# Lalwaniamisha789/Implementation-of-Neural-LDPC-Decoders-with-Degree-Specific-Weight-Sharing-and-RCQ-Quantization

Measured on AMD Instinct MI355X. Metric: decoded codewords/sec at fixed iters; achieved HBM GB/s vs peak, higher is better.
Workload: dtype f32; 1 GPU; (1998,1512) IRA code, BasicMinSumDecoder factor=0.7, fp32, 10 iterations, batch 65536/GPU, SNR 2.0 dB, fixed-iteration flooding decode; graph=ira_1998_1512, n=1998, m=486, edges=6587, batch_per_gpu=65536, global_batch=65536, parallelism=dp1, collective=none

## Files before the change

implementation-of-neural-ldpc-decoders-with-degree-specific-weight-sharing-and-rcq-quantization_amd/_native.py:

```python

from __future__ import annotations

import ctypes as C
import os
import subprocess
import threading
from typing import Optional

import numpy as np

_HERE = os.path.dirname(os.path.abspath(__file__))
LIB_NAME = "libldpc_hip.so"
LIB_PATH = os.environ.get("LDPC_HIP_LIB") or os.path.join(_HERE, LIB_NAME)
CSRC = os.path.join(_HERE, "csrc")
HEADER = os.path.join(os.path.dirname(_HERE), "include", "ldpc_hip.h")
DEBUG_HEADER = os.path.join(os.path.dirname(_HERE), "include", "ldpc_hip_debug.h")

LDPC_F32, LDPC_F64 = 0, 1
C2V_NMS, C2V_RCQ, C2V_OMS = 0, 1, 2
MODE_AUTO, MODE_STREAM, MODE_RESIDENT, MODE_SWEEPS, MODE_GATHER, MODE_PAIR = 0, 1, 2, 3, 4, 5
SCHED_FLOODING, SCHED_LAYERED_REF, SCHED_LAYERED = 0, 1, 2

HIPCC_FLAGS = ["--offload-arch=gfx950", "-O3", "-std=c++17", "-fPIC", "-shared",
               "-ffp-contract=off",
# ... 49 lines not shown
    tmp = target + ".tmp%d" % os.getpid()
    cmd = [hipcc] + HIPCC_FLAGS + [f"-D{d}" for d in defines] + [f"-DLDPC_SRC_HASH={want}", "-o", tmp, srcs[0]]
    res = subprocess.run(cmd, capture_output=True, text=True)
    if verbose or res.returncode != 0:
        print(" ".join(cmd))
        print(res.stdout + res.stderr)
    if res.returncode != 0:
        try:
            os.unlink(tmp)
        except OSError:
            pass
        raise NativeEngineError("hipcc failed:\n" + res.stderr[-4000:])
    os.replace(tmp, target)
    return target


class DecoderDesc(C.Structure):
    _fields_ = [("dtype", C.c_int32), ("c2v_form", C.c_int32), ("iters", C.c_int32),
                ("n_beta_slots", C.c_int32), ("beta", C.c_void_p), ("beta_slot", C.c_void_p),
                ("n_alpha_slots", C.c_int32), ("alpha", C.c_void_p), ("alpha_slot", C.c_void_p),
                ("n_levels", C.c_int32), ("n_quantizers", C.c_int32), ("thresholds", C.c_void_p),
                ("q_of_iter", C.c_void_p),
                ("n_oms_alpha_slots", C.c_int32), ("oms_alpha", C.c_void_p), ("oms_alpha_slot", C.c_void_p),
                ("schedule", C.c_int32)]


PRODUCT_EXPORTS = ("ldpc_graph_create", "ldpc_graph_destroy", "ldpc_graph_info", "ldpc_decoder_create",
                   "ldpc_decoder_set_mode", "ldpc_decoder_info",
                   "ldpc_decoder_set_weights", "ldpc_decoder_destroy", "ldpc_decoder_workspace_bytes",
                   "ldpc_decode", "ldpc_decode_capped", "ldpc_last_error", "ldpc_abi_version", "ldpc_source_hash",
                   "ldpc_train_saved_bytes", "ldpc_train_workspace_bytes", "ldpc_decode_saving", "ldpc_backward",
                   "ldpc_train_joint_workspace_bytes", "ldpc_train_joint")
DEBUG_EXPORTS = ("ldpc_debug_sweep", "ldpc_debug_workspace_layout", "ldpc_debug_resident_c2v", "ldpc_debug_key4",
                 "ldpc_debug_compact_layout")
EXPORTS = PRODUCT_EXPORTS + DEBUG_EXPORTS

_lib = None
_lock = threading.Lock()


def load():
    global _lib
    if _lib is not None:
        return _lib
    with _lock:
        if _lib is not None:
            return _lib
        if not os.path.exists(LIB_PATH):
            raise NativeEngineError(
                f"{LIB_NAME} is not built: run `python -c 'import __graft_entry__ as g; g.build()'` "
                f"(hipcc --offload-arch=gfx950) -- there is no CPU fallback for the decode path")
        if "LDPC_HIP_LIB" not in os.environ and is_stale(LIB_PATH):
            raise NativeEngineError(
                f"{LIB_PATH} was not built from the sources in csrc/ (content hash {built_hash(LIB_PATH)} != "
                f"{source_hash()}): run `python -c 'import __graft_entry__ as g; g.build()'` -- a stale engine is never loaded")
        try:
            lib = C.CDLL(LIB_PATH)
        except OSError as e:
            raise NativeEngineError(f"cannot load {LIB_PATH}: {e}") from e
        vp, i32, i64 = C.c_void_p, C.c_int32, C.c_int64
        lib.ldpc_graph_create.restype = C.c_int
        lib.ldpc_graph_create.argtypes = [C.POINTER(vp), i32, i32, i32, vp, vp]
        lib.ldpc_graph_destroy.restype = None
        lib.ldpc_graph_destroy.argtypes = [vp]
        lib.ldpc_graph_info.restype = C.c_int
        lib.ldpc_graph_info.argtypes = [vp, vp]
        lib.ldpc_decoder_create.restype = C.c_int
        lib.ldpc_decoder_create.argtypes = [C.POINTER(vp), vp, C.POINTER(DecoderDesc)]
        lib.ldpc_decoder_set_mode.restype = C.c_int
        lib.ldpc_decoder_set_mode.argtypes = [vp, i32]
        lib.ldpc_decoder_info.restype = C.c_int
        lib.ldpc_decoder_info.argtypes = [vp, vp]
        lib.ldpc_decoder_set_weights.restype = C.c_int
        lib.ldpc_decoder_set_weights.argtypes = [vp, vp, vp, vp, vp]
        lib.ldpc_decoder_destroy.restype = None
        lib.ldpc_decoder_destroy.argtypes = [vp]
        lib.ldpc_decoder_workspace_bytes.restype = C.c_size_t
        lib.ldpc_decoder_workspace_bytes.argtypes = [vp, i64]
        lib.ldpc_decode.restype = C.c_int
        lib.ldpc_decode.argtypes = [vp, vp, i64, i32, vp, vp, vp, vp, vp, vp, C.c_size_t, vp]
        lib.ldpc_decode_capped.restype = C.c_int
        lib.ldpc_decode_capped.argtypes = [vp, vp, i64, i32, i32, vp, vp, vp, vp, vp, vp, C.c_size_t, vp]
        lib.ldpc_debug_sweep.restype = C.c_int
        lib.ldpc_debug_sweep.argtypes = [vp, i64, i32, i32, vp, C.c_size_t, vp]
        lib.ldpc_debug_workspace_layout.restype = C.c_int
        lib.ldpc_debug_workspace_layout.argtypes = [vp, i64, i32, vp]
        lib.ldpc_debug_key4.restype = C.c_int
        lib.ldpc_debug_key4.argtypes = [vp, i64, C.c_float, vp, vp, vp, vp]
        lib.ldpc_debug_resident_c2v.restype = C.c_int
        lib.ldpc_debug_resident_c2v.argtypes = [vp, vp, i64, i32, i32, vp, vp, vp, vp]
        lib.ldpc_debug_compact_layout.restype = C.c_int
        lib.ldpc_debug_compact_layout.argtypes = [vp, i32, i32, i32, vp, vp, vp, vp, vp]
        lib.ldpc_train_saved_bytes.restype = C.c_size_t
        lib.ldpc_train_saved_bytes.argtypes = [vp, i64]
        lib.ldpc_train_workspace_bytes.restype = C.c_size_t
        lib.ldpc_train_workspace_bytes.argtypes = [vp, i64]
        lib.ldpc_decode_saving.restype = C.c_int
        lib.ldpc_decode_saving.argtypes = [vp, vp, i64, i32, vp, vp, vp, vp, vp, C.c_size_t, vp, C.c_size_t, vp]
        lib.ldpc_backward.restype = C.c_int
        lib.ldpc_backward.argtypes = [vp, vp, C.c_size_t, vp, i64, vp, vp, vp, vp, vp, vp, vp, C.c_size_t, vp]
        lib.ldpc_train_joint_workspace_bytes.restype = C.c_size_t
        lib.ldpc_train_joint_workspace_bytes.argtypes = [vp, i64]
        lib.ldpc_train_joint.restype = C.c_int
        lib.ldpc_train_joint.argtypes = [vp, vp, vp, i64, vp, vp, vp, vp, vp, vp, vp, vp, vp, C.c_size_t, vp]
        lib.ldpc_last_error.restype = C.c_char_p
        lib.ldpc_last_error.argtypes = []
        lib.ldpc_abi_version.restype = C.c_int
        lib.ldpc_abi_version.argtypes = []
        lib.ldpc_source_hash.restype = C.c_char_p
        lib.ldpc_source_hash.argtypes = []
        if lib.ldpc_abi_version() != 1:
            raise NativeEngineError("libldpc_hip.so ABI version mismatch")
        _lib = lib
    return _lib


def check(rc: int, what: str):
    if rc != 0:
        msg = load().ldpc_last_error().decode(errors="replace")
        if rc == -3:
            raise NotImplementedError(f"{what}: {msg}")
        if rc == -1:
            raise ValueError(f"{what}: {msg}")
        raise NativeEngineError(f"{what} failed (rc={rc}): {msg}")

# ... 4 lines not shown
```

implementation-of-neural-ldpc-decoders-with-degree-specific-weight-sharing-and-rcq-quantization_amd/csrc/ldpc_hip.hip:

```cpp
#include "ldpc_kernels.hip"
#include "ldpc_resident.hip"
#include "ldpc_train.hip"
#include "ldpc_layered.hip"

#include <algorithm>
#include <climits>
#include <mutex>
#include <set>
#include <cmath>
#include <cstdarg>
#include <cstdio>
#include <cstdlib>
#include <cstring>
#include <exception>
#include <new>
#include <vector>

#include "../../include/ldpc_hip.h"
#include "../../include/ldpc_hip_debug.h"

using namespace ldpc;

namespace {

// ... 991 lines not shown

void cpt_lane_order(std::vector<int> &var_at, const std::vector<std::vector<int>> &vs, int G)
{
    const int n = (int)vs.size() - 1;
    std::vector<int> order(var_at.size());
    for (size_t q = 0; q < var_at.size(); ++q) order[q] = var_at[q] >= 0 ? var_at[q] : n;
    LaneCost lc{vs, order, 32, 32, G == 2 ? 16 : 32, G == 2 ? 16 : 32};
    std::vector<std::vector<int>> classes(kCptMaxDv + 1);
    for (int q = 0; q < (int)order.size(); ++q) {
        const int d = (int)vs[order[q]].size();
        if (order[q] != n && d > 0 && d <= kCptMaxDv) classes[d].push_back(q);
    }
    classes.erase(std::remove_if(classes.begin(), classes.end(), [](const std::vector<int> &c) { return c.size() < 2; }),
                  classes.end());
    if (classes.empty()) return;
    uint64_t rng = 0x9E3779B97F4A7C15ull;
    auto next = [&]() { rng ^= rng << 13; rng ^= rng >> 7; rng ^= rng << 17; return rng; };
    const long trials = std::min<long>(400000, 150L * n);
    for (long it = 0; it < trials; ++it) {
        const auto &c = classes[next() % classes.size()];
        const int x = c[next() % c.size()], y = c[next() % c.size()];
        if (x / lc.wg == y / lc.wg) continue;
        const int before = lc.around(x, y);
        std::swap(order[x], order[y]);
        if (lc.around(x, y) > before) std::swap(order[x], order[y]);
    }
    for (size_t q = 0; q < var_at.size(); ++q) var_at[q] = order[q] == n ? -1 : order[q];
}

struct ResVCheck { int check, e0, dc, gs; };
int resident_layout(ldpc_decoder *d, const ldpc_decoder_desc *desc, const std::vector<ResVCheck> &vc, int mstride,
                    long long S, int G, ResidentPlan &pl, const CptLayout *cl = nullptr);
void cpt_layout(const ldpc_graph *g, const std::vector<ResVCheck> &vc, long long S, CptLayout &L);
bool cpt_geometry(const ldpc_graph *g, const std::vector<ResVCheck> &vc, long long &Sc);

bool resident_checks(const ldpc_graph *g, std::vector<ResVCheck> &vc)
{
    auto dc_real = [&](int i) { return g->h_check_ptr[i + 1] - g->h_check_ptr[i]; };
    std::vector<int> wide_ids, plain_ids;
    for (int i = 0; i < g->m; ++i) (dc_real(i) > kResSubDegreeCap ? wide_ids : plain_ids).push_back(i);
    auto group_of = [&](int i) { int k = 1; while (k * kResSubDegree < dc_real(i)) k <<= 1; return k; };
    for (int i : wide_ids)
        if (group_of(i) > 64) return false;
    std::stable_sort(wide_ids.begin(), wide_ids.end(), [&](int a, int b) { return group_of(a) > group_of(b); });
    for (int i : wide_ids) {
        const int k = group_of(i), dc = dc_real(i), base = dc / k, rem = dc % k;
        int e = g->h_check_ptr[i];
        for (int j = 0; j < k; ++j) {
            const int len = base + (j < rem ? 1 : 0);
            vc.push_back({i, e, len, k});
            e += len;
        }
    }
    std::stable_sort(plain_ids.begin(), plain_ids.end(), [&](int a, int b) { return dc_real(a) > dc_real(b); });
    for (int i : plain_ids) vc.push_back({i, g->h_check_ptr[i], dc_real(i), 1});
    return true;
}

int build_resident_plan(ldpc_decoder *d, const ldpc_decoder_desc *desc)
{
    const ldpc_graph *g = d->g;
    d->res_ok = false;
    if (g->E == 0 || g->max_dv > 8) return LDPC_OK;
    const bool f64 = d->dtype == LDPC_F64;
    if (f64 && (d->form != LDPC_C2V_NMS || !d->beta_per_check)) return LDPC_OK;
    const int n = g->n;
// ... 25 lines not shown
    }
    const long long S = (long long)max_sub * mstride;
    const int NT = blocks >= 2 ? 512 : 1024;
    if (int rc = resident_layout(d, desc, vc, mstride, S, G, d->res)) return rc;
    d->res_G = G; d->res_NT = NT;
    d->res_lds = res_lds_total((int)S, n, G, resident_alpha_floats(d), d->res.par_words);
    d->res_ok = true;

    d->resc_ok = false;
    long long Sc = 0;
    if (!f64 && G == 2 && NT == kResCptThreads && cpt_geometry(g, vc, Sc)) {
        cpt_layout(g, vc, Sc, d->resc_layout);
        if (int rc = resident_layout(d, desc, vc, kResCptStride, Sc, 2, d->resc, &d->resc_layout)) return rc;
        d->resc_lds = res_cpt_lds_total((int)Sc, 2);
        d->resc_ok = true;
    }
    return LDPC_OK;
}

bool cpt_geometry(const ldpc_graph *g, const std::vector<ResVCheck> &vc, long long &Sc)
{
    const int n = g->n, m = (int)vc.size();
    int max_sub = 0;
    for (const ResVCheck &v : vc) max_sub = std::max(max_sub, v.dc);
    if (m != g->m || m > kResCptStride || n > kResRegVars * kResCptThreads || g->max_dv > kCptMaxDv || max_sub < 1)
        return false;
    int n_top = 0;
    while (n_top < m && vc[n_top].dc == max_sub) ++n_top;
    Sc = (long long)(max_sub - 1) * kResCptStride + n_top;
    int n_hi = 0;
    for (int j = 0; j < n; ++j) n_hi += (g->h_var_ptr[j + 1] - g->h_var_ptr[j]) > 4 ? 1 : 0;
    return Sc * 2 * 4 <= 65535 && (long long)n <= Sc && n_hi <= kResCptThreads &&
           kResCptBlocks * res_cpt_lds_total((int)Sc, 2) <= kLdsBytes;
}

void cpt_layout(const ldpc_graph *g, const std::vector<ResVCheck> &vc, long long S, CptLayout &L)
{
    const int n = g->n, m = (int)vc.size();
    std::vector<int> dv(n);
    for (int j = 0; j < n; ++j) dv[j] = g->h_var_ptr[j + 1] - g->h_var_ptr[j];
    std::vector<int> slot_of_edge(g->E);
    for (int p = 0; p < m; ++p)
        for (int t = 0; t < vc[p].dc; ++t) slot_of_edge[vc[p].e0 + t] = t * kResCptStride + p;
    std::vector<std::vector<int>> vs(n + 1);
    for (int j = 0; j < n; ++j)
        for (int k = 0; k < dv[j]; ++k) vs[j].push_back(slot_of_edge[g->h_csc[g->h_var_ptr[j] + k]]);
    if (!cpt_assign(dv, L) || (long long)L.var_at.size() > S) {
        L.var_at.resize(n);
        for (int j = 0; j < n; ++j) L.var_at[j] = j;
        std::stable_sort(L.var_at.begin(), L.var_at.end(), [&](int a, int b) { return dv[a] > dv[b]; });
    }
    cpt_lane_order(L.var_at, vs, 2);
    cpt_cells(dv, L);
}

int resident_layout(ldpc_decoder *d, const ldpc_decoder_desc *desc, const std::vector<ResVCheck> &vc, int mstride,
                    long long S, int G, ResidentPlan &pl, const CptLayout *cl)
{
    const ldpc_graph *g = d->g;
    const int n = g->n, m = (int)vc.size();
    const bool any_split = m != g->m;
    int max_sub = 0;
    for (const ResVCheck &v : vc) max_sub = std::max(max_sub, v.dc);
    std::vector<int> perm_v(n), pos_v(n);
    for (int j = 0; j < n; ++j) perm_v[j] = j;
    auto dv_of = [&](int j) { return g->h_var_ptr[j + 1] - g->h_var_ptr[j]; };
// ... 22 lines not shown
    std::vector<uint32_t> edge_of_slot((size_t)S, 0xffffffffu);
    bool per_check = true;
    for (int p = 0; p < m; ++p) {
        const ResVCheck &v = vc[p];
        const int first = g->h_check_ptr[v.check];
        dc_s[p] = (uint8_t)v.dc;
        gsz[p] = (uint8_t)v.gs;
        for (int t = 0; t < v.dc; ++t) {
            const int e = v.e0 + t, slot = t * mstride + p;
            edge_of_slot[slot] = (uint32_t)e;
            cvar[slot] = (uint16_t)pos_v[g->h_var_idx[e]];
            bslot[slot] = (uint16_t)desc->beta_slot[e];
            if (desc->beta_slot[e] != desc->beta_slot[first]) per_check = false;
            if (d->form == LDPC_C2V_OMS && desc->oms_alpha) oaslot[slot] = (uint16_t)desc->oms_alpha_slot[e];
        }
        bslot_c[p] = v.dc ? (uint16_t)desc->beta_slot[first] : 0;
    }
    for (int q = 0; q < n_pos; ++q) {
        if (perm_v[q] < 0) continue;
        const int j = perm_v[q], s0 = g->h_var_ptr[j], dv = dv_of(j);
        vmeta[q] = (uint32_t)dv | ((uint32_t)desc->alpha_slot[j] << 8);
        inv[j] = (uint16_t)q;
        uint32_t off[8] = {0, 0, 0, 0, 0, 0, 0, 0};
        for (int k = 0; k < dv; ++k) off[k] = (uint32_t)slot_of_edge[g->h_csc[s0 + k]] * G * 4;
        vslot_lo[q] = make_uint2(off[0] | (off[1] << 16), off[2] | (off[3] << 16));
        vslot_hi[q] = make_uint2(off[4] | (off[5] << 16), off[6] | (off[7] << 16));
        if (dv > 4) n_hi = q + 1;
    }
    pl = ResidentPlan{};
    pl.n = n; pl.m = m; pl.S = (int)S; pl.max_dc = max_sub; pl.max_dv = g->max_dv; pl.mstride = mstride; pl.E = g->E;
    pl.any_split = any_split ? 1 : 0;
    pl.n_hi = n_hi;
    pl.n_pos = n_pos;
    if (cl) std::copy(cl->cell, cl->cell + kCptWaves, pl.vcell);
    pl.par_words = is_pow2(mstride) ? m : 0;
    pl.par_shift = G == 2 ? 3 : 2;
    int rc = plan_upload(d, &pl.dc_s, dc_s);
    if (!rc && any_split) rc = plan_upload(d, &pl.gsz, gsz);
    if (!rc) rc = plan_upload(d, &pl.cvar, cvar);
    if (!rc) rc = plan_upload(d, &pl.bslot, bslot);
    if (!rc && per_check) rc = plan_upload(d, &pl.bslot_c, bslot_c);
    if (!rc && d->form == LDPC_C2V_OMS && desc->oms_alpha) rc = plan_upload(d, &pl.oaslot, oaslot);
    if (!rc) rc = plan_upload(d, &pl.vmeta, vmeta);
    if (!rc) rc = plan_upload(d, &pl.vslot_lo, vslot_lo);
    vslot_hi.resize((size_t)std::max(n_hi, 1));
    if (!rc) rc = plan_upload(d, &pl.vslot_hi, vslot_hi);
    if (!rc) rc = plan_upload(d, &pl.inv_perm_v, inv);
    if (!rc) rc = plan_upload(d, &pl.edge_of_slot, edge_of_slot);
    return rc;
}

int allow_full_lds(const void *kfn, int device)
{
    static std::mutex mu;
    static std::set<std::pair<const void *, int>> done;
    std::lock_guard<std::mutex> lk(mu);
    if (done.count({kfn, device})) return LDPC_OK;
    HIP_TRY(hipFuncSetAttribute(kfn, hipFuncAttributeMaxDynamicSharedMemorySize, (int)kLdsBytes));
    done.insert({kfn, device});
    return LDPC_OK;
}

bool resident_reg_state(const ldpc_decoder *d)
{
    return !d->res.any_split && d->res.n <= kResRegVars * d->res_NT && d->res.n_hi <= d->res_NT;
}

// ... 1001 lines not shown
    const CptLayout *L = &own;
    if (d) {
        if (!d->resc_ok) return fail(LDPC_ERR_UNSUPPORTED, "the decoder has no compact fixed-T plan");
        L = &d->resc_layout;
        n = d->g->n;
    } else {
        ldpc_graph g;
        if (int rc = graph_host_build(&g, n, m, E, check_ptr, var_idx)) return rc;
        std::vector<ResVCheck> vc;
        long long Sc = 0;
        if (!resident_checks(&g, vc) || !cpt_geometry(&g, vc, Sc))
            return fail(LDPC_ERR_UNSUPPORTED, "the graph does not qualify for the compact plan");
        cpt_layout(&g, vc, Sc, own);
    }
    if (pos_of_var) {
        for (int j = 0; j < n; ++j) pos_of_var[j] = -1;
        for (int q = 0; q < (int)L->var_at.size(); ++q)
            if (L->var_at[q] >= 0) pos_of_var[L->var_at[q]] = q;
    }
    if (cells)
        for (int c = 0; c < kCptCells; ++c) cells[c] = (uint8_t)(L->cell[c / kResRegVars] >> (8 * (c % kResRegVars)));
    if (stats) {
        stats[0] = (int32_t)L->var_at.size(); stats[1] = L->worst; stats[2] = L->total; stats[3] = L->mixed;
    }
    return LDPC_OK;
}

int ldpc_debug_compact_layout(const ldpc_decoder *d, int32_t n, int32_t m, int32_t E, const int32_t *check_ptr,
                              const int32_t *var_idx, int32_t *pos_of_var, uint8_t cells[32], int32_t stats[4])
{
    LDPC_NOTHROW(compact_layout_impl(d, n, m, E, check_ptr, var_idx, pos_of_var, cells, stats))
}

int ldpc_debug_resident_c2v(const ldpc_decoder *d, const void *llr, int64_t batch, int32_t early_stop,
                            int32_t max_iterations, void *posterior, int32_t *iterations, void *c2v_out, void *stream)
{
    if (!d || !llr || !posterior || !c2v_out || batch <= 0) return fail(LDPC_ERR_ARG, "bad argument");
    if (!use_resident(d)) return fail(LDPC_ERR_ARG, "the decoder is not on the LDS-resident engine");
    if (d->g->n == 0) return LDPC_OK;
    IterCap cap(max_iterations > 0 ? max_iterations : INT_MAX);
    return decode_resident(d, llr, batch, early_stop, nullptr, posterior, iterations, nullptr, nullptr, c2v_out, stream);
}

int ldpc_debug_sweep(const ldpc_decoder *d, int64_t batch, int32_t which, int32_t iter, void *workspace,
                     size_t workspace_bytes, void *stream)
{
    if (!d || !workspace || batch <= 0) return fail(LDPC_ERR_ARG, "bad argument");
    if (iter < 0 || iter >= d->T) return fail(LDPC_ERR_ARG, "iter outside [0, T)");
    if (use_resident(d) || use_layered_lds(d)) return fail(LDPC_ERR_ARG, "debug sweeps need LDPC_MODE_STREAM");
    const Workspace w = carve(d, batch, workspace);
    if (w.total > workspace_bytes) return fail(LDPC_ERR_WORKSPACE, "workspace too small");
    DeviceGuard guard(d->g->device);
    hipStream_t s = (hipStream_t)stream;
    const bool f64 = d->dtype == LDPC_F64;
    if (use_pair(d) && !f64) {
        if (which == 0 && (iter >= 1 || (w.vec == 4 && pair_q4<4>(d))))
            return w.vec == 1 ? launch_cn_q<1>(d, w, iter, false, s) : launch_cn_q<4>(d, w, iter, false, s);
        if (which != 0 && iter < d->T - 1) return w.vec == 1 ? launch_vn_q<1>(d, w, iter, false, s) : launch_vn_q<4>(d, w, iter, false, s);
    }
    if (use_gather(d) && !f64) {
        char *buf[2] = {w.c2v, w.v2c};
        if (which == 0 && iter >= 1)
            return w.vec == 1 ? launch_gather<1>(d, w, iter, false, buf[(iter - 1) & 1], buf[iter & 1], s)
                              : launch_gather<4>(d, w, iter, false, buf[(iter - 1) & 1], buf[iter & 1], s);
        if (which != 0) {
            Workspace wv = w;
// ... 17 lines not shown
```

implementation-of-neural-ldpc-decoders-with-degree-specific-weight-sharing-and-rcq-quantization_amd/csrc/ldpc_resident.hip:

```cpp
#pragma once

#include "ldpc_kernels.hip"

namespace ldpc {

struct ResidentPlan {
    int n, m, S, max_dc, max_dv;
    int mstride;
    const uint8_t *dc_s;
    const uint8_t *gsz;
    int any_split;
    int par_words;
    int par_shift;
    const uint16_t *cvar;
    const uint16_t *bslot;
    const uint16_t *bslot_c;
    const uint16_t *oaslot;
    const uint32_t *vmeta;
    const uint2 *vslot_lo;
    const uint2 *vslot_hi;
    int n_hi;
    const uint16_t *inv_perm_v;
    int n_pos;
    unsigned vcell[8];
    int E;
    const uint32_t *edge_of_slot;
};

struct ResidentArgs {
    const float *llr;
    long long batch;
    int T, early_stop;
    const float *beta; int n_beta;
    const float *alpha; int n_alpha;
    const float *oms_alpha; int n_oms_alpha;
    const float *thr; int n_levels; const int *q_of_iter;
    int *bits; float *posterior; int *iterations; uint8_t *success; uint8_t *packed;
    int alpha_in_lds;
    int unit_alpha;
    int rcq_zero0;
    void *dbg_c2v;
};

constexpr int kResAlphaMax = 1024;

template <typename X>
__device__ __forceinline__ X lds_load(unsigned byte_off)
{
    constexpr int N = sizeof(X) / sizeof(float);
    typedef float VT __attribute__((ext_vector_type(N)));
    using LP = __attribute__((address_space(3))) const VT *;
    union { VT v; X k; } u;
    u.v = *(LP)(size_t)byte_off;
    return u.k;
}
template <typename X>
__device__ __forceinline__ void lds_store(unsigned byte_off, const X &v)
// ... 86 lines not shown
    group_step<32, G, T>(gs, m1, m2, sg, nz);
}
__device__ __forceinline__ unsigned group_xor(int gs, unsigned x)
{
    unsigned y;
    y = lane_xchg<1>(x);  if (1 < gs) x ^= y;
    y = lane_xchg<2>(x);  if (2 < gs) x ^= y;
    y = lane_xchg<4>(x);  if (4 < gs) x ^= y;
    y = lane_xchg<8>(x);  if (8 < gs) x ^= y;
    y = lane_xchg<16>(x); if (16 < gs) x ^= y;
    y = lane_xchg<32>(x); if (32 < gs) x ^= y;
    return x;
}

__device__ __forceinline__ void res_select4(float &x0, float &x1, float &x2, float &x3, float m1a, float m1b,
                                            uint32_t o1a, uint32_t o2a, uint32_t o1b, uint32_t o2b, uint32_t sign_v)
{
    unsigned long long c0, c1, c2;
    uint32_t t0, t1, t2, t3;
    asm("v_cmp_eq_f32_e64 %8, |%0|, %11\n\t"
        "v_cmp_eq_f32_e64 %9, |%1|, %12\n\t"
        "v_cmp_eq_f32_e64 %10, |%2|, %11\n\t"
        "v_cmp_eq_f32_e64 vcc, |%3|, %12\n\t"
        "v_cndmask_b32_e64 %4, %13, %14, %8\n\t"
        "v_cndmask_b32_e64 %5, %15, %16, %9\n\t"
        "v_cndmask_b32_e64 %6, %13, %14, %10\n\t"
        "v_cndmask_b32_e32 %7, %15, %16, vcc\n\t"
        "v_bitop3_b32 %0, %4, %0, %17 bitop3:0x78\n\t"
        "v_bitop3_b32 %1, %5, %1, %17 bitop3:0x78\n\t"
        "v_bitop3_b32 %2, %6, %2, %17 bitop3:0x78\n\t"
        "v_bitop3_b32 %3, %7, %3, %17 bitop3:0x78"
        : "+v"(x0), "+v"(x1), "+v"(x2), "+v"(x3), "=&v"(t0), "=&v"(t1), "=&v"(t2), "=&v"(t3), "=&s"(c0), "=&s"(c1), "=&s"(c2)
        : "v"(m1a), "v"(m1b), "v"(o1a), "v"(o2a), "v"(o1b), "v"(o2b), "v"(sign_v)
        : "vcc");
}

__device__ __forceinline__ void res_select4_f64(double (&x)[4], double m1, double o1, double o2, uint32_t sign_v)
{
    const unsigned long long b1 = (unsigned long long)__double_as_longlong(o1), b2 = (unsigned long long)__double_as_longlong(o2);
    const uint32_t o1l = (uint32_t)b1, o1h = (uint32_t)(b1 >> 32), o2l = (uint32_t)b2, o2h = (uint32_t)(b2 >> 32);
    uint32_t xh[4], rl[4], rh[4];
#pragma unroll
    for (int i = 0; i < 4; ++i) xh[i] = (uint32_t)((unsigned long long)__double_as_longlong(x[i]) >> 32);
    unsigned long long c0, c1, c2;
    asm("v_cmp_eq_f64_e64 %[c0], |%[x0]|, %[m1]\n\t"
        "v_cmp_eq_f64_e64 %[c1], |%[x1]|, %[m1]\n\t"
        "v_cmp_eq_f64_e64 %[c2], |%[x2]|, %[m1]\n\t"
        "v_cmp_eq_f64_e64 vcc, |%[x3]|, %[m1]\n\t"
        "v_cndmask_b32_e64 %[l0], %[o1l], %[o2l], %[c0]\n\t"
        "v_cndmask_b32_e64 %[h0], %[o1h], %[o2h], %[c0]\n\t"
        "v_cndmask_b32_e64 %[l1], %[o1l], %[o2l], %[c1]\n\t"
        "v_cndmask_b32_e64 %[h1], %[o1h], %[o2h], %[c1]\n\t"
        "v_cndmask_b32_e64 %[l2], %[o1l], %[o2l], %[c2]\n\t"
        "v_cndmask_b32_e64 %[h2], %[o1h], %[o2h], %[c2]\n\t"
        "v_cndmask_b32_e32 %[l3], %[o1l], %[o2l], vcc\n\t"
        "v_cndmask_b32_e32 %[h3], %[o1h], %[o2h], vcc\n\t"
        "v_bitop3_b32 %[h0], %[h0], %[xh0], %[k] bitop3:0x78\n\t"
        "v_bitop3_b32 %[h1], %[h1], %[xh1], %[k] bitop3:0x78\n\t"
        "v_bitop3_b32 %[h2], %[h2], %[xh2], %[k] bitop3:0x78\n\t"
        "v_bitop3_b32 %[h3], %[h3], %[xh3], %[k] bitop3:0x78"
        : [l0] "=&v"(rl[0]), [h0] "=&v"(rh[0]), [l1] "=&v"(rl[1]), [h1] "=&v"(rh[1]), [l2] "=&v"(rl[2]), [h2] "=&v"(rh[2]),
          [l3] "=&v"(rl[3]), [h3] "=&v"(rh[3]), [c0] "=&s"(c0), [c1] "=&s"(c1), [c2] "=&s"(c2)
        : [x0] "v"(x[0]), [x1] "v"(x[1]), [x2] "v"(x[2]), [x3] "v"(x[3]), [m1] "v"(m1), [o1l] "v"(o1l), [o1h] "v"(o1h),
          [o2l] "v"(o2l), [o2h] "v"(o2h), [xh0] "v"(xh[0]), [xh1] "v"(xh[1]), [xh2] "v"(xh[2]), [xh3] "v"(xh[3]), [k] "v"(sign_v)
        : "vcc");
#pragma unroll
    for (int i = 0; i < 4; ++i) x[i] = __longlong_as_double((long long)(((unsigned long long)rh[i] << 32) | rl[i]));
}

template <int G, int FORM, bool BPC, int NL, int MS, typename T, bool SPLIT = false>
__device__ __forceinline__ void res_check_body(const ResidentPlan &pl, unsigned char *smem, int p, int dc,
                                               T b_check, const T *__restrict__ beta_row,
                                               const T *__restrict__ oa_row, const float (&th)[8],
                                               const float *__restrict__ thr, int n_levels, bool rcq_zero0, int gs = 1)
{
    constexpr int kEl = G * (int)sizeof(T);
    const int trip = dc;
    const unsigned stride = (MS > 0 ? (unsigned)MS : (unsigned)pl.mstride) * kEl;
    const unsigned base = (unsigned)p * kEl;
    if constexpr (!std::is_same<T, float>::value) {
        static_assert(FORM == FORM_NMS && BPC, "the fp64 resident engine covers the per-check normalised form");
        using PD = Pack<T, G>;
        T m1[G], m2[G];
        unsigned par[G];
#pragma unroll
        for (int g = 0; g < G; ++g) { m1[g] = inf_of<T>(); m2[g] = inf_of<T>(); par[g] = 0; }
        auto absorb = [&](const PD &v) {
#pragma unroll
            for (int g = 0; g < G; ++g) {
                par[g] ^= signbit_of<T>(v.x[g]);
                T lo, m1n;
                asm("v_min_f64 %0, |%1|, %2" : "=v"(lo) : "v"(v.x[g]), "v"(m2[g]));
                asm("v_min_f64 %0, |%1|, %2" : "=v"(m1n) : "v"(v.x[g]), "v"(m1[g]));
                asm("v_max_f64 %0, %1, %2" : "=v"(m2[g]) : "v"(lo), "v"(m1[g]));
                m1[g] = m1n;
            }
        };
        {
            int t = 0;
            for (; t + 3 < trip; t += 4) {
                const unsigned addr = base + t * stride;
                const PD va = lds_load<PD>(addr), vb = lds_load<PD>(addr + stride);
// ... 131 lines not shown
    for (int t = 0; t < trip; ++t) {
        const unsigned addr = base + t * stride;
        const float b = BPC ? b_check : beta_row[pl.bslot[slot]];
        float oa = 0.0f;
        if (FORM == FORM_OMS && oa_row) oa = oa_row[pl.oaslot[slot]];
        const P v = lds_load<P>(addr);
        P o;
#pragma unroll
        for (int g = 0; g < G; ++g) {
            const float a = __builtin_fabsf(v.x[g]);
            const float raw = (a == m1[g]) ? m2[g] : m1[g];
            const uint32_t sflip = (__float_as_uint(v.x[g]) ^ sacc[g]) & 0x80000000u;
            if (FORM == FORM_NMS) {
                o.x[g] = __uint_as_float(__float_as_uint(b * raw) ^ sflip);
            } else if (FORM == FORM_OMS) {
                const unsigned ownz = (a == 0.0f) ? 1u : 0u;
                const bool nonzero = (nz[g] - ownz) == 0;
                const float d = raw - b;
                const float r = d > 0.0f ? d : 0.0f;
                const float val = r - oa;
                o.x[g] = nonzero ? __uint_as_float(__float_as_uint(val) ^ sflip) : 0.0f;
            } else {
                const float w = __uint_as_float(__float_as_uint(b * raw) ^ sflip);
                const float rec = res_quant_rec<NL>(__builtin_fabsf(w), th, thr, n_levels);
                o.x[g] = flip_sign<float>(rec, (w < 0.0f) ? 1u : 0u);
            }
        }
        lds_store<P>(addr, o);
        slot += sstride;
    }
    }
}

template <int G, int FORM, bool BPC, int NL, int MS, typename T, bool SPLIT>
__device__ __forceinline__ void res_check_phase(const ResidentPlan &pl, unsigned char *smem,
                                                const T *__restrict__ beta_row,
                                                const T *__restrict__ oa_row,
                                                const float *__restrict__ thr, int n_levels, bool rcq_zero0,
                                                int dc_pre, T b_pre, int tid, int nt)
{
    float th[8];
    if (FORM == FORM_RCQ) {
#pragma unroll
        for (int q = 0; q < 8; ++q) th[q] = (q < n_levels) ? thr[q] : __builtin_nanf("");
    }
    int dc = dc_pre;
    T b_check = b_pre;
    for (int p = tid; p < pl.m; p += nt) {
        if (p != tid) {
            dc = pl.dc_s[p];
            b_check = BPC ? beta_row[pl.bslot_c[p]] : (T)0;
        }
        if constexpr (SPLIT) {
            const int gs = pl.gsz[p];
            if (__ballot(gs > 1) != 0ull) {
                res_check_body<G, FORM, BPC, NL, MS, T, true>(pl, smem, p, dc, b_check, beta_row, oa_row, th, thr, n_levels, rcq_zero0, gs);
                continue;
            }
        }
        res_check_body<G, FORM, BPC, NL, MS, T>(pl, smem, p, dc, b_check, beta_row, oa_row, th, thr, n_levels, rcq_zero0);
    }
}

template <int G, int DV, int MODE, typename T>
__device__ __forceinline__ void res_var_body(unsigned char *smem, T *__restrict__ llr_s,
                                             uint8_t *__restrict__ bits_s, int q, const uint4 &slo, const uint4 &shi,
                                             T a, unsigned emask, const ParScatter &ps, Pack<T, G> *lreg)
{
    using P = Pack<T, G>;
    constexpr int ORD = std::is_same<T, float>::value ? 0 : 1;
    P *L = reinterpret_cast<P *>(llr_s);
    const unsigned off[8] = {slo.x, slo.y, slo.z, slo.w, shi.x, shi.y, shi.z, shi.w};
    P x[DV > 0 ? DV : 1];
#pragma unroll
    for (int k = 0; k < DV; ++k) x[k] = lds_load<P>(off[k]);
    P l = lreg ? *lreg : L[q];
    if constexpr (MODE == 0 || MODE == 2 || MODE == 4 || MODE == 6) {
// ... 498 lines not shown
            for (int k = 0; k < kPro; ++k) {
                const int q = q0 + k * nt;
                dvk[k] = 0;
                plo[k] = make_uint2(0, 0);
                phi[k] = make_uint2(0, 0);
                if (q < n) {
                    dvk[k] = (int)(pl.vmeta[q] & 0xffu);
                    plo[k] = pl.vslot_lo[q];
                    if (q < pl.n_hi) phi[k] = pl.vslot_hi[q];
                }
            }
#pragma unroll
            for (int k = 0; k < kPro; ++k) {
                const int q = q0 + k * nt;
                if (q < n) {
                    const uint4 slo = plan_unpack(plo[k]), shi = plan_unpack(phi[k]);
                    const unsigned off[8] = {slo.x, slo.y, slo.z, slo.w, shi.x, shi.y, shi.z, shi.w};
                    P l = L[q];
                    if constexpr (!std::is_same<T, float>::value) {
#pragma unroll
                        for (int g = 0; g < G; ++g) l.x[g] = __builtin_canonicalize(l.x[g]);
                    }
                    if (a.T == 0) {
#pragma unroll
                        for (int g = 0; g < G; ++g) l.x[g] = (T)0;
                    }
#pragma unroll
                    for (int e = 0; e < 8; ++e)
                        if (e < dvk[k]) lds_store<P>(off[e], l);
                }
            }
        }
    }
    const int dc_pre = tid < pl.m ? pl.dc_s[tid] : 0;
    T b_pre = (BPC && tid < pl.m && a.T > 0) ? g_beta[pl.bslot_c[tid]] : (T)0;
    __syncthreads();

    unsigned done = 0;
#pragma unroll
    for (int g = 0; g < G; ++g)
        if (b0 + g >= a.batch) done |= 1u << g;

    for (int it = 0; it < a.T; ++it) {
        const T *beta_row = g_beta + (size_t)it * a.n_beta;
        const T *oa_row = a.oms_alpha ? g_oms_alpha + (size_t)it * a.n_oms_alpha : nullptr;
        const float *thr = FORM == FORM_RCQ ? a.thr + (size_t)a.q_of_iter[it] * a.n_levels : nullptr;
        const T *alpha_lds = a.alpha_in_lds ? alpha_s + it * a.n_alpha : nullptr;
        const T *alpha_glb = g_alpha + (size_t)it * a.n_alpha;
        res_check_phase<G, FORM, BPC, NL, MS, T, SPLIT>(pl, res_smem, beta_row, oa_row, thr, a.n_levels, a.rcq_zero0 != 0,
                                              dc_pre, b_pre, tid, nt);
        if (BPC && tid < pl.m && it + 1 < a.T)
            b_pre = g_beta[(size_t)(it + 1) * a.n_beta + pl.bslot_c[tid]];
        __syncthreads();
        if (ES && !a.posterior) {
            const bool last = it == a.T - 1;
            if (last) res_var_phase<G, 1, T, REG>(pl, res_smem, llr_s, bits_s, (const T *)nullptr, (const T *)nullptr, 0u, tid, nt, st, ps);
            else if (a.unit_alpha) res_var_phase<G, 6, T, REG>(pl, res_smem, llr_s, bits_s, (const T *)nullptr, (const T *)nullptr, 0u, tid, nt, st, ps);
            else res_var_phase<G, 4, T, REG>(pl, res_smem, llr_s, bits_s, alpha_lds, alpha_glb, 0u, tid, nt, st, ps);
            __syncthreads();
            unsigned *su = sh_unsat + (it & 1);
            if (ps.par_off) res_parity_reduce<G, SPLIT>(pl, ps.par_off, su, tid, nt);
            else res_syndrome_phase<G, SPLIT>(pl, bits_s, su, tid, nt);
            __syncthreads();
            const unsigned unsat = *su;
            if (tid == 0) sh_unsat[(it + 1) & 1] = 0;
            const unsigned newly = ~unsat & ~done & kAll;
            if (newly) {
                res_emit_bits<G>(pl, a, bits_s, b0, newly, it + 1, 0u, tid, nt);
                done |= newly;
                if (done == kAll) return;
                __syncthreads();
            }
            continue;
        }
        if (ES) {
            res_var_phase<G, 1, T, REG>(pl, res_smem, llr_s, bits_s, (const T *)nullptr, (const T *)nullptr, 0u, tid, nt, st, ps);
            __syncthreads();
            unsigned *su = sh_unsat + (it & 1);
            if (ps.par_off) res_parity_reduce<G, SPLIT>(pl, ps.par_off, su, tid, nt);
            else res_syndrome_phase<G, SPLIT>(pl, bits_s, su, tid, nt);
            __syncthreads();
            const unsigned unsat = *su;
            if (tid == 0) sh_unsat[(it + 1) & 1] = 0;
// ... 55 lines not shown
```

implementation-of-neural-ldpc-decoders-with-degree-specific-weight-sharing-and-rcq-quantization_amd/engine.py:

```python

from __future__ import annotations

import collections
import ctypes as C
import os
import threading
import weakref
from dataclasses import dataclass
from typing import Optional

import numpy as np
import torch

import _native as nat
from tanner_graph import TannerGraph


@dataclass
class DecodeResult:
    bits: Optional[torch.Tensor]
    posterior: Optional[torch.Tensor]
    iterations: torch.Tensor
    success: torch.Tensor
    packed_bits: Optional[torch.Tensor] = None
# ... 123 lines not shown
        try:
            if getattr(self, "handle", None) is not None and self.handle.value:
                self._lib.ldpc_decoder_destroy(self.handle)
                self.handle = C.c_void_p()
        except Exception:
            pass

    _MODES = {"auto": nat.MODE_AUTO, "stream": nat.MODE_STREAM, "resident": nat.MODE_RESIDENT, "sweeps": nat.MODE_SWEEPS,
              "gather": nat.MODE_GATHER, "pair": nat.MODE_PAIR}

    def set_mode(self, mode: str):
        nat.check(self._lib.ldpc_decoder_set_mode(self.handle, self._MODES[mode]), "ldpc_decoder_set_mode")
        with self._ws_lock:
            self._ws.clear()
        return self

    def info(self) -> dict:
        out = np.zeros(4, dtype=np.int32)
        nat.check(self._lib.ldpc_decoder_info(self.handle, nat.ptr(out)), "ldpc_decoder_info")
        resident = int(out[0]) == nat.MODE_RESIDENT
        if self.schedule == nat.SCHED_FLOODING:
            kernel = "resident" if resident else {3: "sweeps", 4: "cn_gather", 5: "code_pair"}[int(out[0])]
        else:
            paper = self.schedule == nat.SCHED_LAYERED
            kernel = ("layered_paper_lds" if paper else "layered_lds") if resident else \
                     ("layered_rcq<paper>" if paper else "layered_rcq<ref>")
        threads, lds = int(out[2]), int(out[3])
        per_cu = min((160 * 1024) // lds, (32 * 64) // threads) if resident and threads and lds else 0
        stats = np.zeros(4, dtype=np.int32)
        plan = None
        if self._lib.ldpc_debug_compact_layout(self.handle, 0, 0, 0, None, None, None, None, nat.ptr(stats)) == 0:
            plan = {"positions": int(stats[0]), "worst_wave_cost": int(stats[1]), "mean_wave_cost": float(stats[2]) / 8,
                    "mixed_cells": int(stats[3])}
        return {"engine": {2: "resident", 3: "stream", 4: "stream", 5: "stream"}[int(out[0])], "kernel": kernel,
                "stream_form": {2: None, 3: "two-sweeps", 4: "fused-rcq-iteration", 5: "rcq-code-pair"}[int(out[0])],
                "codewords_per_workgroup": int(out[1]),
                "threads_per_workgroup": threads, "lds_bytes": lds, "workgroups_per_cu": per_cu,
                "compact_plan": plan}

    def set_weights(self, beta: Optional[np.ndarray], alpha: Optional[np.ndarray],
                    oms_alpha: Optional[np.ndarray] = None):
        if beta is not None:
            beta = np.ascontiguousarray(beta, dtype=self.np_dtype).reshape(self._table_shapes[0])
        if alpha is not None:
            alpha = np.ascontiguousarray(alpha, dtype=self.np_dtype).reshape(self._table_shapes[1])
        if oms_alpha is not None:
            oms_alpha = np.ascontiguousarray(oms_alpha, dtype=self.np_dtype).reshape(self._table_shapes[2])
        with torch.cuda.device(self.device):
            stream = torch.cuda.current_stream(self.device)
            nat.check(self._lib.ldpc_decoder_set_weights(self.handle, nat.ptr(beta), nat.ptr(alpha),
                                                         nat.ptr(oms_alpha), C.c_void_p(stream.cuda_stream)),
                      "ldpc_decoder_set_weights")
            stream.synchronize()
        if beta is not None:
            self._tables[0] = beta.copy()
        if alpha is not None:
            self._tables[1] = alpha.copy()
        if oms_alpha is not None:
            self._tables[2] = oms_alpha.copy()

    def current_tables(self):
        return tuple(self._tables)

    def workspace_bytes(self, batch: int) -> int:
        return int(self._lib.ldpc_decoder_workspace_bytes(self.handle, int(batch)))

# ... 254 lines not shown
```

include/ldpc_hip_debug.h:

```cpp
#ifndef LDPC_HIP_DEBUG_H
#define LDPC_HIP_DEBUG_H

#include "ldpc_hip.h"

#ifdef __cplusplus
extern "C" {
#endif

int ldpc_debug_sweep(const ldpc_decoder *d, int64_t batch, int32_t which, int32_t iter,
                     void *workspace, size_t workspace_bytes, void *stream);

int ldpc_debug_workspace_layout(const ldpc_decoder *d, int64_t batch, int32_t max_iterations, int64_t out8[8]);

int ldpc_debug_resident_c2v(const ldpc_decoder *d, const void *llr, int64_t batch, int32_t early_stop,
                            int32_t max_iterations, void *posterior, int32_t *iterations, void *c2v_out,
                            void *stream);

int ldpc_debug_compact_layout(const ldpc_decoder *d, int32_t n, int32_t m, int32_t E, const int32_t *check_ptr,
                              const int32_t *var_idx, int32_t *pos_of_var, uint8_t cells[32], int32_t stats[4]);

int ldpc_debug_key4(const float *values, int64_t count, float beta, const float thresholds4[4], uint8_t *keys_float,
                    uint8_t *keys_compare, void *stream);

#ifdef __cplusplus
}
#endif
#endif
```

Baseline: 32.46 million codewords/s.

## Add wave-uniform check-node path with per-wave degree words in compact resident kernel

Precomputes, for each 64-check wave of the compact fixed-iteration plan, a word holding the minimum degree, degree spread and active lane count. The kernel reads this word into a scalar register and, when the wave qualifies, runs a new check-node body whose edge walk is driven by the wave-uniform minimum degree. That body reads edges four at a time with immediate LDS offsets and writes outgoing messages through a fused compare/select/sign-flip asm helper. The aim is to cut per-lane degree branching and address arithmetic in the min-sum check update. In exchange it adds a tail loop over the degree spread, more code paths and inline asm, and a debug export for inspecting the words.

Measured after the change: 33.87 million codewords/s, median of 6. +4.4%, better.

```diff
diff --git a/implementation-of-neural-ldpc-decoders-with-degree-specific-weight-sharing-and-rcq-quantization_amd/_native.py b/implementation-of-neural-ldpc-decoders-with-degree-specific-weight-sharing-and-rcq-quantization_amd/_native.py
--- a/implementation-of-neural-ldpc-decoders-with-degree-specific-weight-sharing-and-rcq-quantization_amd/_native.py
+++ b/implementation-of-neural-ldpc-decoders-with-degree-specific-weight-sharing-and-rcq-quantization_amd/_native.py
@@ -105,7 +105,7 @@
                    "ldpc_train_saved_bytes", "ldpc_train_workspace_bytes", "ldpc_decode_saving", "ldpc_backward",
                    "ldpc_train_joint_workspace_bytes", "ldpc_train_joint")
 DEBUG_EXPORTS = ("ldpc_debug_sweep", "ldpc_debug_workspace_layout", "ldpc_debug_resident_c2v", "ldpc_debug_key4",
-                 "ldpc_debug_compact_layout")
+                 "ldpc_debug_compact_layout", "ldpc_debug_compact_checks")
 EXPORTS = PRODUCT_EXPORTS + DEBUG_EXPORTS
 
 _lib = None
@@ -164,6 +164,8 @@
         lib.ldpc_debug_resident_c2v.argtypes = [vp, vp, i64, i32, i32, vp, vp, vp, vp]
         lib.ldpc_debug_compact_layout.restype = C.c_int
         lib.ldpc_debug_compact_layout.argtypes = [vp, i32, i32, i32, vp, vp, vp, vp, vp]
+        lib.ldpc_debug_compact_checks.restype = C.c_int
+        lib.ldpc_debug_compact_checks.argtypes = [vp, i32, i32, i32, vp, vp, vp]
         lib.ldpc_train_saved_bytes.restype = C.c_size_t
         lib.ldpc_train_saved_bytes.argtypes = [vp, i64]
         lib.ldpc_train_workspace_bytes.restype = C.c_size_t
diff --git a/implementation-of-neural-ldpc-decoders-with-degree-specific-weight-sharing-and-rcq-quantization_amd/csrc/ldpc_hip.hip b/implementation-of-neural-ldpc-decoders-with-degree-specific-weight-sharing-and-rcq-quantization_amd/csrc/ldpc_hip.hip
--- a/implementation-of-neural-ldpc-decoders-with-degree-specific-weight-sharing-and-rcq-quantization_amd/csrc/ldpc_hip.hip
+++ b/implementation-of-neural-ldpc-decoders-with-degree-specific-weight-sharing-and-rcq-quantization_amd/csrc/ldpc_hip.hip
@@ -1047,6 +1047,7 @@
 int resident_layout(ldpc_decoder *d, const ldpc_decoder_desc *desc, const std::vector<ResVCheck> &vc, int mstride,
                     long long S, int G, ResidentPlan &pl, const CptLayout *cl = nullptr);
 void cpt_layout(const ldpc_graph *g, const std::vector<ResVCheck> &vc, long long S, CptLayout &L);
+void cpt_check_words(const std::vector<ResVCheck> &vc, bool select_form, unsigned (&words)[kCptWaves]);
 bool cpt_geometry(const ldpc_graph *g, const std::vector<ResVCheck> &vc, long long &Sc);
 
 bool resident_checks(const ldpc_graph *g, std::vector<ResVCheck> &vc)
@@ -1138,6 +1139,17 @@
     for (int j = 0; j < n; ++j) n_hi += (g->h_var_ptr[j + 1] - g->h_var_ptr[j]) > 4 ? 1 : 0;
     return Sc * 2 * 4 <= 65535 && (long long)n <= Sc && n_hi <= kResCptThreads &&
            kResCptBlocks * res_cpt_lds_total((int)Sc, 2) <= kLdsBytes;
+}
+
+void cpt_check_words(const std::vector<ResVCheck> &vc, bool select_form, unsigned (&words)[kCptWaves])
+{
+    const int m = (int)vc.size();
+    for (int w = 0; w < kCptWaves; ++w) {
+        const int p0 = std::min(64 * w, m), p1 = std::min(p0 + 64, m);
+        int lo = p0 < p1 ? 255 : 0, hi = 0;
+        for (int p = p0; p < p1; ++p) { lo = std::min(lo, vc[p].dc); hi = std::max(hi, vc[p].dc); }
+        words[w] = p0 < p1 ? chk_word(lo, hi, p1 - p0) | (select_form ? 0u : kChkPerLane) : 0u;
+    }
 }
 
 void cpt_layout(const ldpc_graph *g, const std::vector<ResVCheck> &vc, long long S, CptLayout &L)
@@ -1226,7 +1238,11 @@
     pl.any_split = any_split ? 1 : 0;
     pl.n_hi = n_hi;
     pl.n_pos = n_pos;
-    if (cl) std::copy(cl->cell, cl->cell + kCptWaves, pl.vcell);
+    if (cl) {
+        std::copy(cl->cell, cl->cell + kCptWaves, pl.vcell);
+        cpt_check_words(vc, per_check && (d->form == LDPC_C2V_NMS || (d->form == LDPC_C2V_RCQ && d->rcq_zero0)),
+                        pl.ccell);
+    }
     pl.par_words = is_pow2(mstride) ? m : 0;
     pl.par_shift = G == 2 ? 3 : 2;
     int rc = plan_upload(d, &pl.dc_s, dc_s);
@@ -2294,6 +2310,33 @@
     LDPC_NOTHROW(compact_layout_impl(d, n, m, E, check_ptr, var_idx, pos_of_var, cells, stats))
 }
 
+static int compact_checks_impl(const ldpc_decoder *d, int32_t n, int32_t m, int32_t E, const int32_t *check_ptr,
+                               const int32_t *var_idx, uint32_t *words)
+{
+    if (!words) return fail(LDPC_ERR_ARG, "NULL argument");
+    if (d) {
+        if (!d->resc_ok) return fail(LDPC_ERR_UNSUPPORTED, "the decoder has no compact fixed-T plan");
+        std::copy(d->resc.ccell, d->resc.ccell + kCptWaves, words);
+        return LDPC_OK;
+    }
+    ldpc_graph g;
+    if (int rc = graph_host_build(&g, n, m, E, check_ptr, var_idx)) return rc;
+    std::vector<ResVCheck> vc;
+    long long Sc = 0;
+    if (!resident_checks(&g, vc) || !cpt_geometry(&g, vc, Sc))
+        return fail(LDPC_ERR_UNSUPPORTED, "the graph does not qualify for the compact plan");
+    unsigned own[kCptWaves];
+    cpt_check_words(vc, true, own);
+    std::copy(own, own + kCptWaves, words);
+    return LDPC_OK;
+}
+
+int ldpc_debug_compact_checks(const ldpc_decoder *d, int32_t n, int32_t m, int32_t E, const int32_t *check_ptr,
+                              const int32_t *var_idx, uint32_t words[8])
+{
+    LDPC_NOTHROW(compact_checks_impl(d, n, m, E, check_ptr, var_idx, words))
+}
+
 int ldpc_debug_resident_c2v(const ldpc_decoder *d, const void *llr, int64_t batch, int32_t early_stop,
                             int32_t max_iterations, void *posterior, int32_t *iterations, void *c2v_out, void *stream)
 {
diff --git a/implementation-of-neural-ldpc-decoders-with-degree-specific-weight-sharing-and-rcq-quantization_amd/csrc/ldpc_resident.hip b/implementation-of-neural-ldpc-decoders-with-degree-specific-weight-sharing-and-rcq-quantization_amd/csrc/ldpc_resident.hip
--- a/implementation-of-neural-ldpc-decoders-with-degree-specific-weight-sharing-and-rcq-quantization_amd/csrc/ldpc_resident.hip
+++ b/implementation-of-neural-ldpc-decoders-with-degree-specific-weight-sharing-and-rcq-quantization_amd/csrc/ldpc_resident.hip
@@ -23,6 +23,7 @@
     const uint16_t *inv_perm_v;
     int n_pos;
     unsigned vcell[8];
+    unsigned ccell[8];
     int E;
     const uint32_t *edge_of_slot;
 };
@@ -175,6 +176,27 @@
         "v_bitop3_b32 %3, %7, %3, %17 bitop3:0x78"
         : "+v"(x0), "+v"(x1), "+v"(x2), "+v"(x3), "=&v"(t0), "=&v"(t1), "=&v"(t2), "=&v"(t3), "=&s"(c0), "=&s"(c1), "=&s"(c2)
         : "v"(m1a), "v"(m1b), "v"(o1a), "v"(o2a), "v"(o1b), "v"(o2b), "v"(sign_v)
+        : "vcc");
+}
+
+__device__ __forceinline__ void res_select4_out(float (&y)[4], float x0, float x1, float x2, float x3, float m1a, float m1b,
+                                                uint32_t o1a, uint32_t o2a, uint32_t o1b, uint32_t o2b, uint32_t sign_v)
+{
+    unsigned long long c0, c1, c2;
+    asm("v_cmp_eq_f32_e64 %4, |%7|, %11\n\t"
+        "v_cmp_eq_f32_e64 %5, |%8|, %12\n\t"
+        "v_cmp_eq_f32_e64 %6, |%9|, %11\n\t"
+        "v_cmp_eq_f32_e64 vcc, |%10|, %12\n\t"
+        "v_cndmask_b32_e64 %0, %13, %14, %4\n\t"
+        "v_cndmask_b32_e64 %1, %15, %16, %5\n\t"
+        "v_cndmask_b32_e64 %2, %13, %14, %6\n\t"
+        "v_cndmask_b32_e32 %3, %15, %16, vcc\n\t"
+        "v_bitop3_b32 %0, %0, %7, %17 bitop3:0x78\n\t"
+        "v_bitop3_b32 %1, %1, %8, %17 bitop3:0x78\n\t"
+        "v_bitop3_b32 %2, %2, %9, %17 bitop3:0x78\n\t"
+        "v_bitop3_b32 %3, %3, %10, %17 bitop3:0x78"
+        : "=&v"(y[0]), "=&v"(y[1]), "=&v"(y[2]), "=&v"(y[3]), "=&s"(c0), "=&s"(c1), "=&s"(c2)
+        : "v"(x0), "v"(x1), "v"(x2), "v"(x3), "v"(m1a), "v"(m1b), "v"(o1a), "v"(o2a), "v"(o1b), "v"(o2b), "v"(sign_v)
         : "vcc");
 }
 
@@ -211,6 +233,104 @@
     for (int i = 0; i < 4; ++i) x[i] = __longlong_as_double((long long)(((unsigned long long)rh[i] << 32) | rl[i]));
 }
 
+constexpr unsigned kChkPerLane = 0x80000000u;
+__host__ __device__ constexpr unsigned chk_word(int d_lo, int d_hi, int lanes)
+{
+    return (unsigned)d_lo | (unsigned)(d_hi - d_lo) << 8 | (unsigned)lanes << 16 | (d_lo < 4 ? kChkPerLane : 0u);
+}
+__host__ __device__ constexpr int chk_lo(unsigned w) { return (int)(w & 0xffu); }
+__host__ __device__ constexpr int chk_spread(unsigned w) { return (int)(w >> 8 & 0xffu); }
+__host__ __device__ constexpr int chk_lanes(unsigned w) { return (int)(w >> 16 & 0xffu); }
+
+template <typename F>
+__device__ __forceinline__ void res_walk_edges(unsigned base, unsigned stride, int d_lo, int spread, int dc, F &&f)
+{
+    unsigned addr = base;
+#pragma unroll 1
+    for (int t = 0; t + 4 <= d_lo; t += 4) {
+        f(addr, std::integral_constant<int, 4>{});
+        addr += 4 * stride;
+    }
+    if (d_lo & 2) {
+        f(addr, std::integral_constant<int, 2>{});
+        addr += 2 * stride;
+    }
+    if (d_lo & 1) f(addr, std::integral_constant<int, 1>{});
+#pragma unroll 1
+    for (int e = d_lo; e < d_lo + spread; ++e)
+        if (e < dc) f(base + (unsigned)e * stride, std::integral_constant<int, 1>{});
+}
+
+template <int FORM, int NL, int MS>
+__device__ __forceinline__ void res_check_body_uniform(int p, int dc, unsigned cw, float b_check, const float (&th)[8],
+                                                       const float *__restrict__ thr, int n_levels)
+{
+    static_assert(FORM == FORM_NMS || FORM == FORM_RCQ, "forms with two outgoing magnitudes per check");
+    static_assert(MS > 0, "compile-time row stride: the slots of a group are immediate offsets");
+    constexpr int G = 2;
+    using P = Pack<float, G>;
+    constexpr unsigned stride = (unsigned)MS * G * (unsigned)sizeof(float);
+    const unsigned base = (unsigned)p * G * (unsigned)sizeof(float);
+    const int d_lo = chk_lo(cw), spread = chk_spread(cw);
+    float m1[G], m2[G];
+    uint32_t sacc[G];
+    float ninf = -inf_of<float>();
+    asm volatile("" : "+v"(ninf));
+#pragma unroll
+    for (int g = 0; g < G; ++g) {
+        m1[g] = inf_of<float>(); m2[g] = inf_of<float>(); sacc[g] = 0;
+    }
+    res_walk_edges(base, stride, d_lo, spread, dc, [&](unsigned addr, auto kc) {
+        constexpr int K = decltype(kc)::value;
+        P v[K];
+#pragma unroll
+        for (int k = 0; k < K; ++k) v[k] = lds_load<P>(addr + k * stride);
+#pragma unroll
+        for (int k = 0; k < K; ++k) {
+#pragma unroll
+            for (int g = 0; g < G; ++g) {
+                const float a = __builtin_fabsf(v[k].x[g]);
+                sacc[g] ^= __float_as_uint(v[k].x[g]);
+                m2[g] = __builtin_amdgcn_fmed3f(a, m1[g], m2[g]);
+                m1[g] = __builtin_amdgcn_fmed3f(a, m1[g], ninf);
+            }
+        }
+    });
+
+    uint32_t o1[G], o2[G];
+#pragma unroll
+    for (int g = 0; g < G; ++g) {
+        float w1 = b_check * m1[g], w2 = b_check * m2[g];
+        if (FORM == FORM_RCQ) {
+            const float r1 = res_quant_rec<NL>(__builtin_fabsf(w1), th, thr, n_levels);
+            const float r2 = res_quant_rec<NL>(__builtin_fabsf(w2), th, thr, n_levels);
+            w1 = flip_sign<float>(r1, (w1 < 0.0f) ? 1u : 0u);
+            w2 = flip_sign<float>(r2, (w2 < 0.0f) ? 1u : 0u);
+        }
+        const uint32_t par = sacc[g] & 0x80000000u;
+        o1[g] = __float_as_uint(w1) ^ par;
+        o2[g] = __float_as_uint(w2) ^ par;
+        asm volatile("" : "+v"(o1[g]), "+v"(o2[g]));
+    }
+    uint32_t sign_v = 0x80000000u;
+    asm volatile("" : "+v"(sign_v));
+    res_walk_edges(base, stride, d_lo, spread, dc, [&](unsigned addr, auto kc) {
+        constexpr int K = decltype(kc)::value;
+        P v[4];
+#pragma unroll
+        for (int k = 0; k < K; ++k) v[k] = lds_load<P>(addr + k * stride);
+        if constexpr (K & 1) asm volatile("" : "=v"(v[K].x[0]), "=v"(v[K].x[1]));
+#pragma unroll
+        for (int k = 0; k < K; k += 2) {
+            float y[4];
+            res_select4_out(y, v[k].x[0], v[k].x[1], v[k + 1].x[0], v[k + 1].x[1], m1[0], m1[1], o1[0], o2[0], o1[1], o2[1],
+                            sign_v);
+            lds_store<P>(addr + k * stride, P{{y[0], y[1]}});
+            if (k + 1 < K) lds_store<P>(addr + (k + 1) * stride, P{{y[2], y[3]}});
+        }
+    });
+}
+
 template <int G, int FORM, bool BPC, int NL, int MS, typename T, bool SPLIT = false>
 __device__ __forceinline__ void res_check_body(const ResidentPlan &pl, unsigned char *smem, int p, int dc,
                                                T b_check, const T *__restrict__ beta_row,
@@ -408,17 +528,31 @@
     }
 }
 
-template <int G, int FORM, bool BPC, int NL, int MS, typename T, bool SPLIT>
+template <int G, int FORM, bool BPC, int NL, int MS, typename T, bool SPLIT, bool CPT = false>
 __device__ __forceinline__ void res_check_phase(const ResidentPlan &pl, unsigned char *smem,
                                                 const T *__restrict__ beta_row,
                                                 const T *__restrict__ oa_row,
                                                 const float *__restrict__ thr, int n_levels, bool rcq_zero0,
-                                                int dc_pre, T b_pre, int tid, int nt)
+                                                int dc_pre, T b_pre, int tid, int nt, unsigned cw = 0)
 {
     float th[8];
     if (FORM == FORM_RCQ) {
 #pragma unroll
         for (int q = 0; q < 8; ++q) th[q] = (q < n_levels) ? thr[q] : __builtin_nanf("");
+    }
+    if constexpr (CPT && BPC && (FORM == FORM_NMS || FORM == FORM_RCQ)) {
+        static_assert(G == 2 && !SPLIT && std::is_same<T, float>::value, "compact: fp32 codeword pairs, whole checks");
+        asm volatile("" : "+s"(cw));
+        asm volatile("" : "+v"(dc_pre), "+v"(b_pre));
+        if (!(cw & kChkPerLane)) {
+            const int lanes = chk_lanes(cw);
+            if (lanes == 64) res_check_body_uniform<FORM, NL, MS>(tid, dc_pre, cw, b_pre, th, thr, n_levels);
+            else if ((tid & 63) < lanes) res_check_body_uniform<FORM, NL, MS>(tid, dc_pre, cw, b_pre, th, thr, n_levels);
+            return;
+        }
+        if (tid < pl.m)
+            res_check_body<G, FORM, BPC, NL, MS, T>(pl, smem, tid, dc_pre, b_pre, beta_row, oa_row, th, thr, n_levels, rcq_zero0);
+        return;
     }
     int dc = dc_pre;
     T b_check = b_pre;
@@ -983,6 +1117,8 @@
             }
         }
     }
+    unsigned chk_cells = 0;
+    if constexpr (CPT) chk_cells = pl.ccell[__builtin_amdgcn_readfirstlane(tid) >> 6];
     const int dc_pre = tid < pl.m ? pl.dc_s[tid] : 0;
     T b_pre = (BPC && tid < pl.m && a.T > 0) ? g_beta[pl.bslot_c[tid]] : (T)0;
     __syncthreads();
@@ -998,8 +1134,8 @@
         const float *thr = FORM == FORM_RCQ ? a.thr + (size_t)a.q_of_iter[it] * a.n_levels : nullptr;
         const T *alpha_lds = a.alpha_in_lds ? alpha_s + it * a.n_alpha : nullptr;
         const T *alpha_glb = g_alpha + (size_t)it * a.n_alpha;
-        res_check_phase<G, FORM, BPC, NL, MS, T, SPLIT>(pl, res_smem, beta_row, oa_row, thr, a.n_levels, a.rcq_zero0 != 0,
-                                              dc_pre, b_pre, tid, nt);
+        res_check_phase<G, FORM, BPC, NL, MS, T, SPLIT, CPT>(pl, res_smem, beta_row, oa_row, thr, a.n_levels,
+                                                             a.rcq_zero0 != 0, dc_pre, b_pre, tid, nt, chk_cells);
         if (BPC && tid < pl.m && it + 1 < a.T)
             b_pre = g_beta[(size_t)(it + 1) * a.n_beta + pl.bslot_c[tid]];
         __syncthreads();
diff --git a/implementation-of-neural-ldpc-decoders-with-degree-specific-weight-sharing-and-rcq-quantization_amd/engine.py b/implementation-of-neural-ldpc-decoders-with-degree-specific-weight-sharing-and-rcq-quantization_amd/engine.py
--- a/implementation-of-neural-ldpc-decoders-with-degree-specific-weight-sharing-and-rcq-quantization_amd/engine.py
+++ b/implementation-of-neural-ldpc-decoders-with-degree-specific-weight-sharing-and-rcq-quantization_amd/engine.py
@@ -179,6 +179,10 @@
         if self._lib.ldpc_debug_compact_layout(self.handle, 0, 0, 0, None, None, None, None, nat.ptr(stats)) == 0:
             plan = {"positions": int(stats[0]), "worst_wave_cost": int(stats[1]), "mean_wave_cost": float(stats[2]) / 8,
                     "mixed_cells": int(stats[3])}
+            words = np.zeros(8, dtype=np.uint32)
+            nat.check(self._lib.ldpc_debug_compact_checks(self.handle, 0, 0, 0, None, None, nat.ptr(words)),
+                      "ldpc_debug_compact_checks")
+            plan["scalar_check_waves"] = int(np.count_nonzero((words != 0) & (words >> 31 == 0)))
         return {"engine": {2: "resident", 3: "stream", 4: "stream", 5: "stream"}[int(out[0])], "kernel": kernel,
                 "stream_form": {2: None, 3: "two-sweeps", 4: "fused-rcq-iteration", 5: "rcq-code-pair"}[int(out[0])],
                 "codewords_per_workgroup": int(out[1]),
diff --git a/include/ldpc_hip_debug.h b/include/ldpc_hip_debug.h
--- a/include/ldpc_hip_debug.h
+++ b/include/ldpc_hip_debug.h
@@ -19,6 +19,9 @@
 int ldpc_debug_compact_layout(const ldpc_decoder *d, int32_t n, int32_t m, int32_t E, const int32_t *check_ptr,
                               const int32_t *var_idx, int32_t *pos_of_var, uint8_t cells[32], int32_t stats[4]);
 
+int ldpc_debug_compact_checks(const ldpc_decoder *d, int32_t n, int32_t m, int32_t E, const int32_t *check_ptr,
+                              const int32_t *var_idx, uint32_t words[8]);
+
 int ldpc_debug_key4(const float *values, int64_t count, float beta, const float thresholds4[4], uint8_t *keys_float,
                     uint8_t *keys_compare, void *stream);
 
```
